# dmsuehir/unet_distributed

Hardware: AMD Instinct MI355X
Metric: images/sec (whole node) 2D UNet BraTS 128×128×4 at 1/2/4/8 MI355X; Dice parity (higher is better)
Workload: dtype bf16; 1 GPU; model=unet2d-transposed (base 32, depth 4, 7760385 params), global_batch=1024, per_gpu_batch=1024, img_size=128, in_channels=4, parallelism=dp1, backend=native

## Files before the change

unet_distributed_amd/csrc/kernels/conv_epilogue.h:

```cpp
#pragma once
#include "common.h"
#include "conv_params.h"

namespace unet {

struct PixCoord {
  int n, d, h, w;
};

__device__ __forceinline__ PixCoord decompose(int q, int OD, int OH, int OW) {
  PixCoord c;
  c.w = q % OW;
  int t = q / OW;
  c.h = t % OH;
  t /= OH;
  c.d = t % OD;
  c.n = t / OD;
  return c;
}

enum { EPI_GENERIC = 0, EPI_FWD = 1, EPI_DGRAD = 2, EPI_STATS = 3, EPI_DGRAD_NORM = 4 };

template <int BM, int BN, int NTHR = 256>
constexpr int epi_lds_bytes() {
// ... 35 lines not shown
  return EPI_GENERIC;
}

template <int WM>
struct LinearTiles {
  __device__ static int base(int wm, int i) { return wm * WM + i * 16; }
};
template <int W, int RW, int TC, int NCS>
struct StripTiles {
  __device__ static int base(int wave, int i) {
    return ((wave / NCS) * RW + i / TC) * W + (wave % NCS) * 16 * TC + (i % TC) * 16;
  }
};

constexpr int kWaitVm0 = 0x0f70, kWaitLgkm0 = 0xc07f;
__device__ __forceinline__ void lds_barrier() {
  asm volatile("" ::: "memory");
  __builtin_amdgcn_s_waitcnt(kWaitLgkm0);
  __builtin_amdgcn_s_barrier();
  asm volatile("" ::: "memory");
}

template <int TN>
struct EpiConst {
  float bias[TN][4];
  float hw[8];
  float hb;
};

struct HeadWsum {
// ... 4 lines not shown
  float t[8];
  bool on;
};

template <int BM, int BN, int NTHR>
__device__ __forceinline__ void epi_mask_bits_load(const ConvFwdParams& p, const int m0, const int n0, const int tid,
                                                   uint32_t (&mb)[BM * (BN / 8) / NTHR]) {
  constexpr int CPR = BN / 8, NIT = BM * CPR / NTHR, RPI = NTHR / CPR;
  static_assert(BM * CPR % NTHR == 0 && NTHR % CPR == 0, "whole chunk passes");
  const int co = n0 + (tid % CPR) * 8, ml0 = tid / CPR;
#pragma unroll
  for (int it = 0; it < NIT; ++it)
    mb[it] = ((const uint8_t*)p.mask1)[((size_t)(m0 + ml0 + it * RPI) * p.D1 + co) >> 3];
}

template <int BM, int BN, int WM, int WN, int TM, int TN, int NTHR, int EPI = EPI_GENERIC,
          class MapM = LinearTiles<WM>, int SEGW = 0, int TROW = 0>
__device__ __forceinline__ HeadWsum conv_epilogue(const ConvFwdParams p, f32x4 (&acc)[TM][TN], char* smem,
                                                  const int m0, const int n0, const int M, const int wm,
                                                  const int wn, const int lane, const int tid,
                                                  const int pitch = 0, const int col0 = 0, const int stat_row = 0,
                                                  const EpiConst<TN>* ec = nullptr, const HeadT ht = HeadT{},
                                                  const uint32_t* pmb = nullptr) {
  HeadWsum hws;
#pragma unroll
  for (int k = 0; k < 3; ++k)
#pragma unroll
    for (int e = 0; e < 8; ++e) hws.s[k][e] = 0.f;
  hws.u = hws.v = hws.w = 0.f;
  auto qof = [&](int ml) -> int {
    if constexpr (SEGW > 0) return (m0 + ml / SEGW) * pitch + col0 + (ml % SEGW);
    else return m0 + ml;
  };
  constexpr bool ESWZ = BN == 32;
  constexpr int EPI_STRIDE = ESWZ ? 64 : (BN + 4) * 2;
  auto eoff = [](const int ml, const int chunk) -> int {
    return ESWZ ? ml * 64 + 16 * (chunk ^ ((ml >> 2) & 3)) : ml * EPI_STRIDE + 16 * chunk;
  };
  auto ehalf = [](const int ml, const int nl) -> int {
    return ESWZ ? ml * 64 + 16 * ((nl >> 3) ^ ((ml >> 2) & 3)) + ((2 * (nl & 7)) ^ (8 * ((ml >> 1) & 1)))
                : ml * EPI_STRIDE + 2 * nl;
  };
  auto eread = [&](const int ml, const int chunk) -> u32x4 {
    if constexpr (ESWZ) {
// ... 192 lines not shown
      *(u32x4*)(dst + (size_t)q * p.Cout + n) = gv;
      unpack8(gv, g);
#pragma unroll
      for (int e = 0; e < 8; ++e) {
        s1[e] += g[e];
        s2[e] = fmaf(g[e], z[e], s2[e]);
      }
    }
    stats_out(s1, s2, cb);
    return hws;
  }
  if constexpr (EPI == EPI_DGRAD && NCHUNK % NTHR == 0 && NTHR % CPR == 0) {
    constexpr int NIT = NCHUNK / NTHR, RPI = NTHR / CPR;
    const int cb = tid % CPR, ml0 = tid / CPR;
    const int n = n0 + cb * 8;
    const bool side1 = n < p.D1;
    const int rs = side1 ? p.D1 : p.Cout - p.D1;
    const int co = side1 ? n : n - p.D1;
    h16* dst = (h16*)(side1 ? p.dst1 : p.dst2);
    const h16* mk = (const h16*)(side1 ? p.mask1 : p.mask2);
    const bool mbit = (p.mask_bits >> (side1 ? 0 : 1)) & 1;
    u32x4 mv[NIT];
    uint32_t mb[NIT];
    if (mk && pmb) {
#pragma unroll
      for (int it = 0; it < NIT; ++it) mb[it] = pmb[it];
    } else if (mk) {
#pragma unroll
      for (int it = 0; it < NIT; ++it) {
        const int q = qof(ml0 + it * RPI);
        if (q < M) {
          if (mbit)
            mb[it] = ((const uint8_t*)mk)[((size_t)q * rs + co) >> 3];
          else
            mv[it] = *(const u32x4*)(mk + (size_t)q * rs + co);
        }
      }
    }
    const bool route = !pmb && p.route_gy != nullptr, d3 = p.OD > 1;
    u32x4 rg[NIT];
    uint32_t rc[NIT], rk[NIT];
    if (route) {
      const int cpp = p.Cout >> 3;
#pragma unroll
      for (int it = 0; it < NIT; ++it) {
        const int q = qof(ml0 + it * RPI);
        if (q < M) {
          const size_t pq = route_pix(p, q, rk[it]);
          rc[it] = p.pool_code[pq * cpp + (n >> 3)];
          rg[it] = *(const u32x4*)((const h16*)p.route_gy + pq * p.Cout + n);
        }
      }
    }
#pragma unroll
    for (int it = 0; it < NIT; ++it) {
      const int ml = ml0 + it * RPI;
      const int q = qof(ml);
      if (q >= M) continue;
      u32x4 v = eread(ml, cb);
      if (mk) v = (mbit || pmb) ? keep_bits(v, mb[it]) : keep_pos(v, mv[it]);
      if (route) {
        float o[8], gg[8];
        unpack8(v, o);
        unpack8(rg[it], gg);
        const uint32_t cw = rc[it];
#pragma unroll
        for (int e = 0; e < 8; ++e)
          if (route_hit(cw, e, rk[it], d3)) o[e] += gg[e];
        v = pack8(o);
      }
      *(u32x4*)(dst + (size_t)q * rs + co) = v;
    }
    return hws;
  }
  const int Dt = kShuffle ? (p.Cout >> p.shuffle) : 0;
  constexpr bool kHeadable = EPI == EPI_FWD && BN == 32 && NTHR % CPR == 0;
  const bool kHead = kHeadable && p.head_w != nullptr;
  float hw[8], hb = 0.f;
  constexpr int HIT = kHeadable ? NCHUNK / NTHR : 1;
  static_assert(!kHeadable || (NCHUNK % NTHR == 0 && HIT % CPR == 0 && HIT <= 8), "fused head tiling");
  float hz[HIT];
  int hq[HIT];
#pragma unroll
  for (int k = 0; k < HIT; ++k) {
    hz[k] = 0.f;
    hq[k] = M;
  }
  if (kHeadable && kHead) {
#pragma unroll
    for (int e = 0; e < 8; ++e) hw[e] = ec ? ec->hw[e] : p.head_w[(tid % CPR) * 8 + e];
    hb = ec ? ec->hb : p.head_b[0];
  }
  constexpr int NITER = (NCHUNK + NTHR - 1) / NTHR;
  constexpr int UNR = kHeadable ? NITER : 2;
#pragma unroll UNR
  for (int it = 0; it < NITER; ++it) {
    const int c = tid + it * NTHR;
    if (NCHUNK % NTHR && c >= NCHUNK) break;
    const int ml = c / CPR, cb = c % CPR;
    const int q = qof(ml);
    if (q >= M) continue;
    const int n = n0 + cb * 8;
    u32x4 v = eread(ml, cb);
    size_t off;
    h16* dst;
    const void* mk;
    bool mbit = false;
    if (EPI == EPI_FWD || EPI == EPI_STATS) {
      off = (size_t)q * p.Cout + n;
      dst = (h16*)p.dst1;
      mk = nullptr;
    } else if (kShuffle) {
      const int tap = n / Dt, co = n - tap * Dt;
      const PixCoord pc = decompose(q, p.OD, p.OH, p.OW);
      int td = 0, th, tw;
      if (p.shuffle == 3) {
// ... 13 lines not shown
      mbit = p.mask_bits & 1;
    } else if (n < p.D1) {
      off = (size_t)q * p.D1 + n;
      dst = (h16*)p.dst1;
      mk = p.mask1;
      mbit = p.mask_bits & 1;
    } else {
      off = (size_t)q * (p.Cout - p.D1) + (n - p.D1);
      dst = (h16*)p.dst2;
      mk = p.mask2;
      mbit = (p.mask_bits >> 1) & 1;
    }
    if (EPI != EPI_FWD && EPI != EPI_STATS && mk) {
      v = mbit ? keep_bits(v, ((const uint8_t*)mk)[off >> 3]) : keep_pos(v, *(const u32x4*)((const h16*)mk + off));
    }
    if (!(kHeadable && kHead && p.head_nostore)) *(u32x4*)(dst + off) = v;
    if (EPI == EPI_FWD && p.relu_bits) p.relu_bits[off >> 3] = (uint8_t)pos_bits_relu(v);
    if (G && p.relu_bits) p.relu_bits[off >> 3] = (uint8_t)pos_bits(v);
    if constexpr (kHeadable) {
      if (kHead) {
        float f[8];
        unpack8(v, f);
        float z = 0.f;
#pragma unroll
        for (int e = 0; e < 8; ++e) z += f[e] * hw[e];
        z += __shfl_xor(z, 1, 64);
        z += __shfl_xor(z, 2, 64);
        hz[it] = z + hb;
        hq[it] = q;
        if (ht.on) {
          const float zl = z + hb;
          const float pr = __builtin_amdgcn_rcpf(1.f + __expf(-zl));
          const float tv = ht.t[it];
          const float vv = pr * (1.f - pr), uu = tv * vv, ww = pr - tv;
#pragma unroll
          for (int e = 0; e < 8; ++e) {
            hws.s[0][e] = fmaf(uu, f[e], hws.s[0][e]);
            hws.s[1][e] = fmaf(vv, f[e], hws.s[1][e]);
            hws.s[2][e] = fmaf(ww, f[e], hws.s[2][e]);
          }
          if (cb == 0) {
            hws.u += uu;
            hws.v += vv;
            hws.w += ww;
          }
// ... 1 lines not shown
      }
    }
  }
  if constexpr (kHeadable) {
    if (kHead) {
      const int cb = tid % CPR;
#pragma unroll
      for (int k = 0; k < HIT / CPR; ++k) {
        float z = hz[CPR * k];
        int q = hq[CPR * k];
#pragma unroll
        for (int r = 1; r < CPR; ++r) {
          z = cb == r ? hz[CPR * k + r] : z;
          q = cb == r ? hq[CPR * k + r] : q;
        }
        if (q < M) p.head_logit[q] = z;
      }
    }
  }
  if constexpr (EPI == EPI_FWD && TROW > 0 && (BM / TROW) % 2 == 0 && TROW % 2 == 0) {
    if (p.pool_dst) {
      constexpr int PC = TROW / 2, NP = (BM / TROW / 2) * PC * CPR;
      const int Wp = p.OW >> 1, cpp = p.Cout >> 3;
      h16* pdst = (h16*)p.pool_dst;
      for (int k = tid; k < NP; k += NTHR) {
        const int cb = k % CPR, pp = k / CPR;
        const int pr = pp / PC, pc = pp - pr * PC;
        const int ml00 = 2 * pr * TROW + 2 * pc;
        const int q00 = qof(ml00);
        if (q00 >= M) continue;
        int32_t key[8];
#pragma unroll
        for (int e = 0; e < 8; ++e) key[e] = INT32_MIN;
#pragma unroll
        for (int kk = 0; kk < 4; ++kk) {
          const int ml = ml00 + (kk >> 1) * TROW + (kk & 1);
          const u32x4 v = eread(ml, cb);
#pragma unroll
          for (int e = 0; e < 4; ++e) {
            key[2 * e] = max(key[2 * e], (int32_t)((v[e] << 16) | (3u - kk)));
            key[2 * e + 1] = max(key[2 * e + 1], (int32_t)((v[e] & 0xffff0000u) | (3u - kk)));
          }
        }
        uint32_t w = 0;
        u32x4 mv;
#pragma unroll
        for (int e = 0; e < 8; ++e)
          w |= ((3u - ((uint32_t)key[e] & 3u)) << (2 * e)) | ((key[e] > 3 ? 1u : 0u) << (24 + e));
#pragma unroll
        for (int e = 0; e < 4; ++e)
          mv[e] = ((uint32_t)key[2 * e] >> 16) | ((uint32_t)key[2 * e + 1] & 0xffff0000u);
        const int grow = q00 / p.OW, gcol = q00 - grow * p.OW;
        const size_t pq = (size_t)(grow >> 1) * Wp + (gcol >> 1);
        *(u32x4*)(pdst + pq * p.Cout + n0 + cb * 8) = mv;
        p.pool_code[pq * cpp + (n0 >> 3) + cb] = w;
      }
    }
  }
  return hws;
}

}
```

unet_distributed_amd/csrc/kernels/conv_win.h:

```cpp
#pragma once
#include "common.h"
#include "conv_params.h"
#include "conv_epilogue.h"
#include "head_grad.h"
#include <type_traits>

namespace unet {

enum { GEO_2D = 0, GEO_SEG = 1, GEO_3D = 2 };

inline int win_bn(const ConvFwdParams& p) {
  if (p.tile == 12) return 64;
  if (p.tile == 6) return 32;
  const int W = p.OW > 128 ? 128 : p.OW;
  return (p.Cout % 64 == 0 && W <= 64 && !p.head_w) ? 64 : 32;
}
inline int win_bm(const ConvFwdParams& p) {
  const int W = p.OW > 128 ? 128 : p.OW;
  return (W == 16 || win_bn(p) == 64) ? 256 : 512;
}
inline int win_rows(const ConvFwdParams& p) {
  const int W = p.OW > 128 ? 128 : p.OW;
  return win_bm(p) / W;
}
// ... 523 lines not shown
#pragma unroll
    for (int k = 0; k < 3; ++k)
#pragma unroll
      for (int e = 0; e < 8; ++e) red[wave * 100 + k * 32 + lane * 8 + e] = hws.s[k][e];
  }
  if (lane == 0) {
    red[wave * 100 + 96] = hws.u;
    red[wave * 100 + 97] = hws.v;
    red[wave * 100 + 98] = hws.w;
    red[wave * 100 + 99] = 0.f;
  }
  __syncthreads();
  if (tid < 100) row[tid] = (red[tid] + red[100 + tid]) + (red[200 + tid] + red[300 + tid]);
}

template <int EPI, int XF, int GEO = GEO_2D>
__global__ void __launch_bounds__(NTHR, 2) conv_win_pf_kernel(const ConvFwdParams p) {
  static_assert(XF == 0 || (XF == 3 && EPI == EPI_DGRAD && GEO == GEO_2D) || (XF == 1 && GEO == GEO_2D),
                "plain source, head-on-load data gradient or normalise on load");
  static_assert(GEO == GEO_2D || GEO == GEO_SEG, "2D rows");
  constexpr bool SEG = GEO == GEO_SEG;
  constexpr int W = 128, R = 4, BM = 512, BN = 32, ROWB = PF_ROWB;
  constexpr int TC = 2, NCS = 4, RW = 4, TM = RW * TC, TN = 2, WMP = BM / 4;
  using Map = StripTiles<W, RW, TC, NCS>;
  __shared__ __attribute__((aligned(1024))) char smem[PF_XB + PF_WB];
  char* Xs = smem;
  char* Ws = smem + PF_XB;
  const int tid = threadIdx.x, lane = tid & 63, wave = __builtin_amdgcn_readfirstlane(tid >> 6);
  const int H = p.OH;
  const int Wf = SEG ? p.OW : W;
  const int nseg = SEG ? p.OW / W : 1;
  const int rows_total = p.N * H;
  const int M = rows_total * Wf;
  const int nwin = rows_total / R * nseg;
// ... 3 lines not shown
  constexpr int OOB = 0x7fffffff;
  const char* src = (const char*)p.src1;

  u32x4 hv[PF_CPT], ev = {0u, 0u, 0u, 0u};
  const int gl_t = tid * 16;
  const int lds_t = (1 + (tid >> 2)) * 64 + 16 * ((tid & 3) ^ (((1 + (tid >> 2)) >> 1) & 3));
  constexpr int NSL = 6 * PF_HWP, HJ = (NSL + NTHR - 1) / NTHR;
  float hpr[HJ], htv[HJ];
  uint32_t hbits[HJ];
  HeadGradCtx hctx{};
  if constexpr (XF == 3) hctx = head_grad_ctx(p.hg);
  float xan[8], xbn[8];
  int pf_g0 = 0;
  bool pf_top = false, pf_bot = false;
  constexpr bool HWS = EPI == EPI_FWD && !SEG;
  float tnext[HWS ? 8 : 1];
  auto load_halo = [&](const int w) {
    const int tmw = p.rev ? nwin - 1 - w : w;
    const int g0 = (tmw / nseg) * R, col0 = (tmw % nseg) * W;
    if constexpr (HWS) {
      if (p.head_ws) {
#pragma unroll
        for (int it = 0; it < 8; ++it) tnext[it] = bits2f(((const uint16_t*)p.head_t)[g0 * W + (tid >> 2) + 64 * it]);
      }
    }
    if constexpr (XF == 3) {
      const bool top_in = (g0 % H) != 0, bot_in = ((g0 + R) % H) != 0;
#pragma unroll
      for (int j = 0; j < HJ; ++j) {
        const int sl = tid + NTHR * j;
        const int hr = sl / PF_HWP, hc = sl - hr * PF_HWP;
        const int gr = g0 - 1 + hr, col = hc - 1;
        const bool ok = sl < NSL && (hr > 0 || top_in) && (hr < R + 1 || bot_in) &&
                        (unsigned)gr < (unsigned)rows_total && (unsigned)col < (unsigned)W;
        const int pix = ok ? gr * W + col : 0;
        hpr[j] = p.hg.prob[pix];
        htv[j] = bits2f(((const uint16_t*)p.hg.t)[pix]);
        hbits[j] = ok ? ((const uint32_t*)p.hg.bits)[pix] : 0u;
// ... 4 lines not shown
    const bool top_in = (g0 % H) != 0, bot_in = ((g0 + R) % H) != 0;
    if constexpr (XF == 1) {
      const size_t cs = (size_t)(g0 / H) * p.xcs + (tid & 3) * 8;
#pragma unroll
      for (int e = 0; e < 8; ++e) {
        xan[e] = p.xa[cs + e];
        xbn[e] = p.xb[cs + e];
      }
      pf_g0 = g0;
      pf_top = top_in;
      pf_bot = bot_in;
    }
    const __amdgpu_buffer_rsrc_t rs =
        __builtin_amdgcn_make_buffer_rsrc((void*)(src + (size_t)grow0 * Wf * 64), (short)0, OOB, 0x00020000);
    const int rowoff = ((g0 - 1 - grow0) * Wf + col0) * 64;
#pragma unroll
    for (int c = 0; c < PF_CPT; ++c) {
      const int hr = c >> 1;
      const bool ok = (hr > 0 || top_in) && (hr < R + 1 || bot_in) && (unsigned)(g0 - 1 + hr) < (unsigned)rows_total;
      hv[c] = __builtin_amdgcn_raw_buffer_load_b128(rs, ok ? rowoff + hr * Wf * 64 + (c & 1) * 4096 + gl_t : OOB, 0, 0);
    }
    if constexpr (SEG) {
      const int hr = tid >> 3, col = ((tid >> 2) & 1) ? col0 + W : col0 - 1;
      const bool ok = tid < 48 && (hr > 0 || top_in) && (hr < R + 1 || bot_in) &&
                      (unsigned)(g0 - 1 + hr) < (unsigned)rows_total && (unsigned)col < (unsigned)Wf;
      ev = __builtin_amdgcn_raw_buffer_load_b128(
          rs, ok ? ((g0 - 1 + hr - grow0) * Wf + col) * 64 + (tid & 3) * 16 : OOB, 0, 0);
    }
  };
  auto store_halo = [&]() {
    if constexpr (XF == 3) {
#pragma unroll
      for (int j = 0; j < HJ; ++j) {
        const int sl = tid + NTHR * j;
        if (sl >= NSL) continue;
// ... 24 lines not shown
          unpack8(v, f);
#pragma unroll
          for (int e = 0; e < 8; ++e) f[e] = fmaxf(fmaf(xan[e], f[e], xbn[e]), 0.f);
          v = pack8(f);
          if (p.xout && hr >= 1 && hr <= R)
            *(u32x4*)((h16*)p.xout + ((size_t)gr * W + (tid >> 2) + 64 * (c & 1)) * 32 + (tid & 3) * 8) = v;
        }
        *(u32x4*)(Xs + lds_t + hr * ROWB + (c & 1) * 4096) = v;
      }
    } else {
#pragma unroll
      for (int c = 0; c < PF_CPT; ++c) *(u32x4*)(Xs + lds_t + (c >> 1) * ROWB + (c & 1) * 4096) = hv[c];
    }
    if (tid < 48) *(u32x4*)(Xs + (tid >> 3) * ROWB + ((tid >> 2) & 1) * 129 * 64 + 16 * (tid & 3)) = ev;
  };
  load_halo(w_lo);
  {
    const __amdgpu_buffer_rsrc_t rsw = __builtin_amdgcn_make_buffer_rsrc((void*)p.wgt, (short)0, OOB, 0x00020000);
    const int lslot = lane >> 2;
    const int lchunk = (lane & 3) ^ ((lslot >> 1) & 3);
    const int wl = (lslot * p.Kpad + lchunk * 8) * 2;
    constexpr int WI = 9 * BN / 16;
#pragma unroll
    for (int q = 0; q < (WI + 3) / 4; ++q) {
      const int k = wave + 4 * q;
      if (k < WI) {
        const int tap = k / (BN / 16), nb = (k % (BN / 16)) * 16;
        __builtin_amdgcn_raw_ptr_buffer_load_lds(rsw, (__attribute__((address_space(3))) void*)(Ws + k * 1024), 16,
                                                 (nb * p.Kpad + tap * 32) * 2 + wl, 0, 0, 0);
      }
// ... 4 lines not shown
#pragma unroll
  for (int j = 0; j < TN; ++j)
#pragma unroll
    for (int r = 0; r < 4; ++r)
      ec.bias[j][r] = (EPI != EPI_DGRAD && EPI != EPI_DGRAD_NORM && p.bias) ? p.bias[16 * j + 4 * fsub + r] : 0.f;
#pragma unroll
  for (int e = 0; e < 8; ++e) ec.hw[e] = (EPI == EPI_FWD && p.head_w) ? p.head_w[(tid % 4) * 8 + e] : 0.f;
  ec.hb = (EPI == EPI_FWD && p.head_w) ? p.head_b[0] : 0.f;
  HeadWsum hws;
#pragma unroll
  for (int k = 0; k < 3; ++k)
#pragma unroll
    for (int e = 0; e < 8; ++e) hws.s[k][e] = 0.f;
  hws.u = hws.v = hws.w = 0.f;
  HeadT ht;
  ht.on = HWS && p.head_ws;
#pragma unroll
  for (int it = 0; it < 8; ++it) ht.t[it] = HWS ? tnext[it] : 0.f;
  store_halo();
  __syncthreads();

  const int r0 = (wave / NCS) * RW, c0 = (wave % NCS) * 16 * TC;
  int xbase[3];
#pragma unroll
  for (int dw = 0; dw < 3; ++dw) {
    const int hc = fr + dw;
    xbase[dw] = r0 * ROWB + c0 * 64 + hc * 64 + 16 * (fsub ^ ((hc >> 1) & 3));
  }
  const int wbase = fr * 64 + 16 * (fsub ^ ((fr >> 1) & 3));
  for (int w = w_lo; w < w_hi; ++w) {
    const int tm = p.rev ? nwin - 1 - w : w;
    const int g0 = (tm / nseg) * R, col0 = (tm % nseg) * W;
    if (w + 1 < w_hi) load_halo(w + 1);
    f32x4 acc[TM][TN];
#pragma unroll
    for (int i = 0; i < TM; ++i)
#pragma unroll
      for (int j = 0; j < TN; ++j) acc[i][j] = (f32x4){0.f, 0.f, 0.f, 0.f};
#pragma unroll
    for (int dw = 0; dw < 3; ++dw) {
      h16x8 wf[3][TN];
#pragma unroll
      for (int dh = 0; dh < 3; ++dh)
#pragma unroll
        for (int j = 0; j < TN; ++j) wf[dh][j] = *(const h16x8*)(Ws + ((3 * dh + dw) * BN + 16 * j) * 64 + wbase);
#pragma unroll
      for (int hr = 0; hr < RW + 2; ++hr) {
#pragma unroll
// ... 2 lines not shown
#pragma unroll
          for (int dh = 0; dh < 3; ++dh) {
            const int ri = hr - dh;
            if (ri < 0 || ri >= RW) continue;
#pragma unroll
            for (int j = 0; j < TN; ++j) acc[ri * TC + ci][j] = mfma16(wf[dh][j], xf, acc[ri * TC + ci][j]);
          }
        }
      }
    }
    __syncthreads();
    if constexpr (SEG)
      conv_epilogue<BM, BN, WMP, BN, TM, TN, NTHR, EPI, Map, W, W>(p, acc, smem, g0, 0, M, wave, 0, lane, tid, Wf,
                                                                    col0, tm, &ec);
    else {
      const HeadWsum r = conv_epilogue<BM, BN, WMP, BN, TM, TN, NTHR, EPI, Map, 0, W>(
          p, acc, smem, g0 * W, 0, M, wave, 0, lane, tid, 0, 0, tm, &ec, ht);
      if constexpr (HWS) {
#pragma unroll
        for (int k = 0; k < 3; ++k)
#pragma unroll
          for (int e = 0; e < 8; ++e) hws.s[k][e] += r.s[k][e];
        hws.u += r.u;
        hws.v += r.v;
        hws.w += r.w;
      }
    }
    if (w + 1 < w_hi) {
      __syncthreads();
      store_halo();
      if constexpr (HWS) {
#pragma unroll
        for (int it = 0; it < 8; ++it) ht.t[it] = tnext[it];
      }
      __syncthreads();
    }
  }
  if constexpr (EPI == EPI_FWD && !SEG) {
    if (p.head_ws) head_ws_store(hws, smem, wave, lane, tid, p.head_ws + (size_t)blockIdx.x * 100);
  }
}

template <int W, bool CONCAT, int EPI, bool DZ = false>
__global__ void __launch_bounds__(NTHR, 2) conv_win_cp_kernel(const ConvFwdParams p) {
  constexpr int BN = 64, BM = 256, R = BM / W, HR = R + 2;
  constexpr int HWP = W + 4, ROWB = HWP * 64;
  constexpr int NSLOT = HR * HWP;
  constexpr int XB = (NSLOT + 15) / 16 * 1024, WB = 9 * BN * 64;
  constexpr int XG = (NSLOT * 4 + NTHR - 1) / NTHR;
  constexpr int WG = 9 * BN * 4 / NTHR;
  constexpr int EPIB = (EPI == EPI_STATS || EPI == EPI_DGRAD_NORM) ? epi_lds_bytes<BM, BN>() : BM * (BN + 4) * 2;
  constexpr int KB = DZ ? 3 * CP_DZ_MAXC * 4 : 0;
  constexpr int LDS_BYTES = (XB + WB + KB > EPIB) ? XB + WB + KB : EPIB;
  constexpr int WMP = BM / 4, TM = WMP / 16, TN = BN / 16;
// ... 347 lines not shown
    default: UNET_LAUNCH((conv_win_cp128_kernel<GEO, CC, EPI_GENERIC>), dim3(grid), dim3(NTHR), 0, s, p); break;     \
  }
  if (cc) {
    CP1_EPI(true)
  } else {
    CP1_EPI(false)
  }
#undef CP1_EPI
  return launch_status();
}

hipError_t launch_win_cp128(const ConvFwdParams& p, hipStream_t s) {
  return (p.KD == 3) ? launch_win_cp128_g<GEO_3D>(p, s) : launch_win_cp128_g<GEO_2D>(p, s);
}

template <int KS, int EPI>
__global__ void __launch_bounds__(NTHR, 2) conv_win_pfu_kernel(const ConvFwdParams p) {
  static_assert(EPI == EPI_FWD || EPI == EPI_STATS, "persistent tconv-on-load epilogues");
  constexpr int W = 128, R = 2, HR = R + 2, BM = 256, BN = 32, ROWB = PF_ROWB;
  constexpr int TC = 2, NCS = 4, RW = 2, TM = RW * TC, TN = 2, WMP = BM / 4;
  constexpr int CW = W / 2, PB = CW / 16, Cc = KS * 32;
  constexpr int XB = HR * ROWB, WB = 9 * BN * 64;
  static_assert(BM * 64 + 4 * 2 * BN * 4 <= XB, "epilogue staging aliases the halo image");
  using Map = StripTiles<W, RW, TC, NCS>;
  __shared__ __attribute__((aligned(1024))) char smem[XB + 2 * WB];
  char* Xs = smem;
  char* Wu = smem + XB;
  char* Wk = smem + XB + WB;
  const int tid = threadIdx.x, lane = tid & 63, wave = __builtin_amdgcn_readfirstlane(tid >> 6);
  const int fsub = lane >> 4, fr = lane & 15;
  const int H = p.OH;
  const int rows_total = p.N * H;
  const int M = rows_total * W;
// ... 34 lines not shown
  }
  float bs[8];
#pragma unroll
  for (int i = 0; i < 8; ++i) bs[i] = p.ut.b[8 * fsub + i];
  EpiConst<TN> ec;
#pragma unroll
  for (int j = 0; j < TN; ++j)
#pragma unroll
    for (int r = 0; r < 4; ++r) ec.bias[j][r] = p.bias ? p.bias[16 * j + 4 * fsub + r] : 0.f;
#pragma unroll
  for (int e = 0; e < 8; ++e) ec.hw[e] = 0.f;
  ec.hb = 0.f;

  h16x8 xb[PB][KS];
  bool xin = false;
  auto load_coarse = [&](const int w) {
    const int g0 = (p.rev ? nwin - 1 - w : w) * R;
    const bool top_in = (g0 % H) != 0, bot_in = ((g0 + R) % H) != 0;
    const int hr = wave;
    xin = (hr > 0 || top_in) && (hr < R + 1 || bot_in) && (unsigned)(g0 - 1 + hr) < (unsigned)rows_total;
    const int crow = (g0 >> 1) - 1 + cq;
    const h16* rp = (const h16*)p.ut.x + ((size_t)(xin ? crow : 0) * CW + fr) * Cc + 8 * fsub;
#pragma unroll
    for (int pb = 0; pb < PB; ++pb)
#pragma unroll
      for (int ks = 0; ks < KS; ++ks) xb[pb][ks] = *(const h16x8*)(rp + (size_t)(16 * pb) * Cc + 32 * ks);
  };
  u32x4 sv[8];
  uint32_t sok = 0;
  float s2a[8], s2b[8];
  const int lds_t = (1 + (tid >> 2)) * 64 + 16 * ((tid & 3) ^ (((1 + (tid >> 2)) >> 1) & 3));
  auto load_skip = [&](const int w) {
    const int g0 = (p.rev ? nwin - 1 - w : w) * R;
    const int grow0 = (g0 / H) * H;
    const bool top_in = (g0 % H) != 0, bot_in = ((g0 + R) % H) != 0;
    const __amdgpu_buffer_rsrc_t rs =
        __builtin_amdgcn_make_buffer_rsrc((void*)((const char*)p.src2 + (size_t)grow0 * W * 64), (short)0, OOB, 0x00020000);
    const int rowoff = (g0 - 1 - grow0) * W * 64;
    sok = 0;
#pragma unroll
    for (int c = 0; c < 8; ++c) {
      const int hr = c >> 1;
      const bool ok = (hr > 0 || top_in) && (hr < R + 1 || bot_in) && (unsigned)(g0 - 1 + hr) < (unsigned)rows_total;
      sok |= (ok ? 1u : 0u) << c;
      sv[c] = __builtin_amdgcn_raw_buffer_load_b128(rs, ok ? rowoff + hr * W * 64 + (c & 1) * 4096 + tid * 16 : OOB, 0, 0);
    }
    if (p.x2a) {
      const size_t cs = (size_t)(g0 / H) * p.x2cs + (tid & 3) * 8;
#pragma unroll
      for (int e = 0; e < 8; ++e) {
        s2a[e] = p.x2a[cs + e];
        s2b[e] = p.x2b[cs + e];
      }
    }
  };
  const int tsel = (fr >> 2) & 1;
  auto form_u = [&]() {
    char* xrow = Xs + wave * ROWB;
#pragma unroll
    for (int pb = 0; pb < PB; ++pb) {
      u32x4 pk[2] = {(u32x4){0u, 0u, 0u, 0u}, (u32x4){0u, 0u, 0u, 0u}};
      if (xin) {
// ... 6 lines not shown
            for (int ks = 0; ks < KS; ++ks) a = mfma16(wa[tw][j][ks], xb[pb][ks], a);
            pk[tw][2 * j] = pack2h(a[0] + bs[4 * j], a[1] + bs[4 * j + 1]);
            pk[tw][2 * j + 1] = pack2h(a[2] + bs[4 * j + 2], a[3] + bs[4 * j + 3]);
          }
      }
#pragma unroll
      for (int s = 0; s < 2; ++s) {
        const int tw = s ^ tsel;
        const int hc = 2 * (16 * pb + fr) + tw + 1;
        *(u32x4*)(xrow + hc * 64 + 16 * (fsub ^ ((hc >> 1) & 3))) = tw ? pk[1] : pk[0];
      }
    }
    if (lane < 8) *(u32x4*)(xrow + ((lane >> 2) ? W + 1 : 0) * 64 + 16 * (lane & 3)) = (u32x4){0u, 0u, 0u, 0u};
  };
  auto store_skip = [&]() {
    if (p.x2a) {
#pragma unroll
      for (int c = 0; c < 8; ++c) {
        if (!((sok >> c) & 1u)) continue;
        float f[8];
        unpack8(sv[c], f);
#pragma unroll
        for (int e = 0; e < 8; ++e) f[e] = fmaxf(fmaf(s2a[e], f[e], s2b[e]), 0.f);
        sv[c] = pack8(f);
      }
    }
#pragma unroll
    for (int c = 0; c < 8; ++c) *(u32x4*)(Xs + lds_t + (c >> 1) * ROWB + (c & 1) * 4096) = sv[c];
    if (tid < 32) *(u32x4*)(Xs + (tid >> 3) * ROWB + ((tid >> 2) & 1) * 129 * 64 + 16 * (tid & 3)) = (u32x4){0u, 0u, 0u, 0u};
  };

// ... 20 lines not shown
        for (int ci = 0; ci < TC; ++ci) {
          const h16x8 xf = *(const h16x8*)(Xs + xbase[dw] + hr * ROWB + ci * 16 * 64);
#pragma unroll
          for (int dh = 0; dh < 3; ++dh) {
            const int ri = hr - dh;
            if (ri < 0 || ri >= RW) continue;
#pragma unroll
            for (int j = 0; j < TN; ++j) acc[ri * TC + ci][j] = mfma16(wf[dh][j], xf, acc[ri * TC + ci][j]);
          }
        }
      }
    }
  };
  load_coarse(w_lo);
  load_skip(w_lo);
  for (int w = w_lo; w < w_hi; ++w) {
    const int tm = p.rev ? nwin - 1 - w : w;
    const int g0 = tm * R;
#pragma unroll
    for (int i = 0; i < TM; ++i)
#pragma unroll
      for (int j = 0; j < TN; ++j) acc[i][j] = (f32x4){0.f, 0.f, 0.f, 0.f};
    form_u();
    if (w + 1 < w_hi) load_coarse(w + 1);
    __syncthreads();
    chunk_mfmas(Wu);
    __syncthreads();
    store_skip();
    if (w + 1 < w_hi) load_skip(w + 1);
    __syncthreads();
    chunk_mfmas(Wk);
    __syncthreads();
    conv_epilogue<BM, BN, WMP, BN, TM, TN, NTHR, EPI, Map, 0, W>(p, acc, smem, g0 * W, 0, M, wave, 0, lane, tid, 0, 0,
                                                                  tm, &ec);
    __syncthreads();
  }
}

hipError_t launch_win_pfu(const ConvFwdParams& p, hipStream_t s) {
  const int grid = win_grid(p);
  const bool st = conv_epi_mode(p) == EPI_STATS;
  if (p.ut.C == 64 && st)
    UNET_LAUNCH((conv_win_pfu_kernel<2, EPI_STATS>), dim3(grid), dim3(NTHR), 0, s, p);
  else if (p.ut.C == 64)
    UNET_LAUNCH((conv_win_pfu_kernel<2, EPI_FWD>), dim3(grid), dim3(NTHR), 0, s, p);
  else if (st)
    UNET_LAUNCH((conv_win_pfu_kernel<1, EPI_STATS>), dim3(grid), dim3(NTHR), 0, s, p);
  else
    UNET_LAUNCH((conv_win_pfu_kernel<1, EPI_FWD>), dim3(grid), dim3(NTHR), 0, s, p);
  return launch_status();
}

hipError_t launch_win_pf(const ConvFwdParams& p, hipStream_t s) {
  const int grid = win_grid(p);
  if (p.OW > 128) {
    switch (conv_epi_mode(p)) {
      case EPI_FWD: UNET_LAUNCH((conv_win_pf_kernel<EPI_FWD, 0, GEO_SEG>), dim3(grid), dim3(NTHR), 0, s, p); break;
      case EPI_DGRAD: UNET_LAUNCH((conv_win_pf_kernel<EPI_DGRAD, 0, GEO_SEG>), dim3(grid), dim3(NTHR), 0, s, p); break;
// ... 1 lines not shown
      case EPI_DGRAD_NORM:
        UNET_LAUNCH((conv_win_pf_kernel<EPI_DGRAD_NORM, 0, GEO_SEG>), dim3(grid), dim3(NTHR), 0, s, p);
        break;
      default: UNET_LAUNCH((conv_win_pf_kernel<EPI_GENERIC, 0, GEO_SEG>), dim3(grid), dim3(NTHR), 0, s, p); break;
    }
    return launch_status();
  }
  if (p.xform) {
    if (conv_epi_mode(p) == EPI_STATS)
      UNET_LAUNCH((conv_win_pf_kernel<EPI_STATS, 1>), dim3(grid), dim3(NTHR), 0, s, p);
    else if (conv_epi_mode(p) == EPI_GENERIC)
      UNET_LAUNCH((conv_win_pf_kernel<EPI_GENERIC, 1>), dim3(grid), dim3(NTHR), 0, s, p);
    else
      return hipErrorInvalidValue;
    return launch_status();
  }
  switch (conv_epi_mode(p)) {
    case EPI_FWD: UNET_LAUNCH((conv_win_pf_kernel<EPI_FWD, 0>), dim3(grid), dim3(NTHR), 0, s, p); break;
    case EPI_DGRAD:
      if (p.hg.prob)
        UNET_LAUNCH((conv_win_pf_kernel<EPI_DGRAD, 3>), dim3(grid), dim3(NTHR), 0, s, p);
      else
        UNET_LAUNCH((conv_win_pf_kernel<EPI_DGRAD, 0>), dim3(grid), dim3(NTHR), 0, s, p);
      break;
    case EPI_STATS: UNET_LAUNCH((conv_win_pf_kernel<EPI_STATS, 0>), dim3(grid), dim3(NTHR), 0, s, p); break;
    case EPI_DGRAD_NORM: UNET_LAUNCH((conv_win_pf_kernel<EPI_DGRAD_NORM, 0>), dim3(grid), dim3(NTHR), 0, s, p); break;
    default: UNET_LAUNCH((conv_win_pf_kernel<EPI_GENERIC, 0>), dim3(grid), dim3(NTHR), 0, s, p); break;
  }
  return launch_status();
}
// ... 188 lines not shown
```

Before: 49940 images/sec.

## Specialise windowed conv epilogues into fixed compile-time forms for common layer configs

Adds a FORM template parameter that fixes at compile time which epilogue features (ReLU bitmask, 2x2 pool, fused head, gradient routing) are active and asserts full tiles, removing runtime pointer checks and bounds tests. The host picks these specialised kernels when the parameters match. The prefetch loop now always issues loads, dummy and clamped via a max-offset trick, so control flow has no branches, and head targets are loaded later as packed 32-bit words. It adds more kernel instantiations and assumes whole windows, which risks correctness if the dispatch conditions miss a case, and the extra dummy loads cost some bandwidth.

```diff
diff --git a/unet_distributed_amd/csrc/kernels/conv_epilogue.h b/unet_distributed_amd/csrc/kernels/conv_epilogue.h
--- a/unet_distributed_amd/csrc/kernels/conv_epilogue.h
+++ b/unet_distributed_amd/csrc/kernels/conv_epilogue.h
@@ -73,6 +73,8 @@
 };
 
 constexpr int kWaitVm0 = 0x0f70, kWaitLgkm0 = 0xc07f;
+constexpr int vm_wait(const int n) { return (n & 15) | ((n >> 4) << 14) | 0x0f70; }
+static_assert(vm_wait(0) == kWaitVm0 && vm_wait(63) == 0xcf7f, "gfx9 s_waitcnt encoding");
 __device__ __forceinline__ void lds_barrier() {
   asm volatile("" ::: "memory");
   __builtin_amdgcn_s_waitcnt(kWaitLgkm0);
@@ -107,8 +109,18 @@
     mb[it] = ((const uint8_t*)p.mask1)[((size_t)(m0 + ml0 + it * RPI) * p.D1 + co) >> 3];
 }
 
+enum { EF_FULL = 1, EF_FIXED = 2, EF_BITS = 4, EF_POOL = 8, EF_HEAD = 16, EF_ROUTE = 32 };
+template <int BM, int BN, int NTHR, int EPI, int TROW, int FORM>
+constexpr int epi_store_count() {
+  if (!(FORM & EF_FIXED)) return 0;
+  constexpr int CPR = BN / 8, NIT = BM * CPR / NTHR;
+  if (EPI == EPI_DGRAD) return NIT;
+  return ((FORM & EF_HEAD) ? NIT / CPR : NIT) + ((FORM & EF_BITS) ? NIT : 0) +
+         ((FORM & EF_POOL) ? 2 * ((BM / TROW / 2) * (TROW / 2) * CPR / NTHR) : 0);
+}
+
 template <int BM, int BN, int WM, int WN, int TM, int TN, int NTHR, int EPI = EPI_GENERIC,
-          class MapM = LinearTiles<WM>, int SEGW = 0, int TROW = 0>
+          class MapM = LinearTiles<WM>, int SEGW = 0, int TROW = 0, int FORM = 0>
 __device__ __forceinline__ HeadWsum conv_epilogue(const ConvFwdParams p, f32x4 (&acc)[TM][TN], char* smem,
                                                   const int m0, const int n0, const int M, const int wm,
                                                   const int wn, const int lane, const int tid,
@@ -121,6 +133,9 @@
 #pragma unroll
     for (int e = 0; e < 8; ++e) hws.s[k][e] = 0.f;
   hws.u = hws.v = hws.w = 0.f;
+  constexpr bool FULL = (FORM & EF_FULL) != 0, FIXED = (FORM & EF_FIXED) != 0;
+  static_assert(!FIXED || (FULL && SEGW == 0 && (EPI == EPI_FWD || EPI == EPI_DGRAD)), "fixed forms: whole 2D windows");
+  static_assert(!FIXED || EPI != EPI_DGRAD || (FORM & EF_BITS), "fixed data-gradient forms take a 1-bit mask");
   auto qof = [&](int ml) -> int {
     if constexpr (SEGW > 0) return (m0 + ml / SEGW) * pitch + col0 + (ml % SEGW);
     else return m0 + ml;
@@ -343,22 +358,22 @@
     constexpr int NIT = NCHUNK / NTHR, RPI = NTHR / CPR;
     const int cb = tid % CPR, ml0 = tid / CPR;
     const int n = n0 + cb * 8;
-    const bool side1 = n < p.D1;
+    const bool side1 = FIXED || n < p.D1;
     const int rs = side1 ? p.D1 : p.Cout - p.D1;
     const int co = side1 ? n : n - p.D1;
     h16* dst = (h16*)(side1 ? p.dst1 : p.dst2);
     const h16* mk = (const h16*)(side1 ? p.mask1 : p.mask2);
-    const bool mbit = (p.mask_bits >> (side1 ? 0 : 1)) & 1;
+    const bool mbit = FIXED || ((p.mask_bits >> (side1 ? 0 : 1)) & 1);
     u32x4 mv[NIT];
     uint32_t mb[NIT];
-    if (mk && pmb) {
+    if ((FIXED || mk) && pmb) {
 #pragma unroll
       for (int it = 0; it < NIT; ++it) mb[it] = pmb[it];
-    } else if (mk) {
+    } else if (FIXED || mk) {
 #pragma unroll
       for (int it = 0; it < NIT; ++it) {
         const int q = qof(ml0 + it * RPI);
-        if (q < M) {
+        if (FULL || q < M) {
           if (mbit)
             mb[it] = ((const uint8_t*)mk)[((size_t)q * rs + co) >> 3];
           else
@@ -366,7 +381,8 @@
         }
       }
     }
-    const bool route = !pmb && p.route_gy != nullptr, d3 = p.OD > 1;
+    const bool route = FIXED ? (FORM & EF_ROUTE) != 0 : (!pmb && p.route_gy != nullptr);
+    const bool d3 = !FIXED && p.OD > 1;
     u32x4 rg[NIT];
     uint32_t rc[NIT], rk[NIT];
     if (route) {
@@ -374,7 +390,7 @@
 #pragma unroll
       for (int it = 0; it < NIT; ++it) {
         const int q = qof(ml0 + it * RPI);
-        if (q < M) {
+        if (FULL || q < M) {
           const size_t pq = route_pix(p, q, rk[it]);
           rc[it] = p.pool_code[pq * cpp + (n >> 3)];
           rg[it] = *(const u32x4*)((const h16*)p.route_gy + pq * p.Cout + n);
@@ -385,9 +401,9 @@
     for (int it = 0; it < NIT; ++it) {
       const int ml = ml0 + it * RPI;
       const int q = qof(ml);
-      if (q >= M) continue;
+      if (!FULL && q >= M) continue;
       u32x4 v = eread(ml, cb);
-      if (mk) v = (mbit || pmb) ? keep_bits(v, mb[it]) : keep_pos(v, mv[it]);
+      if (FIXED || mk) v = (mbit || pmb) ? keep_bits(v, mb[it]) : keep_pos(v, mv[it]);
       if (route) {
         float o[8], gg[8];
         unpack8(v, o);
@@ -404,7 +420,11 @@
   }
   const int Dt = kShuffle ? (p.Cout >> p.shuffle) : 0;
   constexpr bool kHeadable = EPI == EPI_FWD && BN == 32 && NTHR % CPR == 0;
-  const bool kHead = kHeadable && p.head_w != nullptr;
+  static_assert(!FIXED || EPI != EPI_FWD || kHeadable || !(FORM & EF_HEAD), "fixed head form: a headable tile");
+  const bool kHead = FIXED ? (FORM & EF_HEAD) != 0 : (kHeadable && p.head_w != nullptr);
+  const bool kNoStore = FIXED ? (FORM & EF_HEAD) != 0 : (kHeadable && kHead && p.head_nostore);
+  const bool kBitsF = FIXED ? (FORM & EF_BITS) != 0 : (p.relu_bits != nullptr);
+  const bool kHws = FIXED ? (FORM & EF_HEAD) != 0 : ht.on;
   float hw[8], hb = 0.f;
   constexpr int HIT = kHeadable ? NCHUNK / NTHR : 1;
   static_assert(!kHeadable || (NCHUNK % NTHR == 0 && HIT % CPR == 0 && HIT <= 8), "fused head tiling");
@@ -428,7 +448,7 @@
     if (NCHUNK % NTHR && c >= NCHUNK) break;
     const int ml = c / CPR, cb = c % CPR;
     const int q = qof(ml);
-    if (q >= M) continue;
+    if (!FULL && q >= M) continue;
     const int n = n0 + cb * 8;
     u32x4 v = eread(ml, cb);
     size_t off;
@@ -472,21 +492,27 @@
     if (EPI != EPI_FWD && EPI != EPI_STATS && mk) {
       v = mbit ? keep_bits(v, ((const uint8_t*)mk)[off >> 3]) : keep_pos(v, *(const u32x4*)((const h16*)mk + off));
     }
-    if (!(kHeadable && kHead && p.head_nostore)) *(u32x4*)(dst + off) = v;
-    if (EPI == EPI_FWD && p.relu_bits) p.relu_bits[off >> 3] = (uint8_t)pos_bits_relu(v);
+    if (!kNoStore) *(u32x4*)(dst + off) = v;
+    if (EPI == EPI_FWD && kBitsF) p.relu_bits[off >> 3] = (uint8_t)pos_bits_relu(v);
     if (G && p.relu_bits) p.relu_bits[off >> 3] = (uint8_t)pos_bits(v);
     if constexpr (kHeadable) {
       if (kHead) {
         float f[8];
         unpack8(v, f);
         float z = 0.f;
-#pragma unroll
-        for (int e = 0; e < 8; ++e) z += f[e] * hw[e];
+        if constexpr (FIXED) {
+#pragma clang fp contract(off)
+#pragma unroll
+          for (int e = 0; e < 8; ++e) z += f[e] * hw[e];
+        } else {
+#pragma unroll
+          for (int e = 0; e < 8; ++e) z += f[e] * hw[e];
+        }
         z += __shfl_xor(z, 1, 64);
         z += __shfl_xor(z, 2, 64);
         hz[it] = z + hb;
-        hq[it] = q;
-        if (ht.on) {
+        if constexpr (!FULL) hq[it] = q;
+        if (kHws) {
           const float zl = z + hb;
           const float pr = __builtin_amdgcn_rcpf(1.f + __expf(-zl));
           const float tv = ht.t[it];
@@ -518,21 +544,22 @@
           z = cb == r ? hz[CPR * k + r] : z;
           q = cb == r ? hq[CPR * k + r] : q;
         }
-        if (q < M) p.head_logit[q] = z;
+        if constexpr (FULL) q = qof((tid + (CPR * k + cb) * NTHR) / CPR);
+        if (FULL || q < M) p.head_logit[q] = z;
       }
     }
   }
   if constexpr (EPI == EPI_FWD && TROW > 0 && (BM / TROW) % 2 == 0 && TROW % 2 == 0) {
-    if (p.pool_dst) {
+    if (FIXED ? (FORM & EF_POOL) != 0 : p.pool_dst != nullptr) {
       constexpr int PC = TROW / 2, NP = (BM / TROW / 2) * PC * CPR;
       const int Wp = p.OW >> 1, cpp = p.Cout >> 3;
       h16* pdst = (h16*)p.pool_dst;
-      for (int k = tid; k < NP; k += NTHR) {
+      auto pool_px = [&](const int k) {
         const int cb = k % CPR, pp = k / CPR;
         const int pr = pp / PC, pc = pp - pr * PC;
         const int ml00 = 2 * pr * TROW + 2 * pc;
         const int q00 = qof(ml00);
-        if (q00 >= M) continue;
+        if (!FULL && q00 >= M) return;
         int32_t key[8];
 #pragma unroll
         for (int e = 0; e < 8; ++e) key[e] = INT32_MIN;
@@ -558,6 +585,12 @@
         const size_t pq = (size_t)(grow >> 1) * Wp + (gcol >> 1);
         *(u32x4*)(pdst + pq * p.Cout + n0 + cb * 8) = mv;
         p.pool_code[pq * cpp + (n0 >> 3) + cb] = w;
+      };
+      if constexpr (FULL && NP % NTHR == 0) {
+#pragma unroll
+        for (int kp = 0; kp < NP / NTHR; ++kp) pool_px(tid + kp * NTHR);
+      } else {
+        for (int k = tid; k < NP; k += NTHR) pool_px(k);
       }
     }
   }
diff --git a/unet_distributed_amd/csrc/kernels/conv_win.h b/unet_distributed_amd/csrc/kernels/conv_win.h
--- a/unet_distributed_amd/csrc/kernels/conv_win.h
+++ b/unet_distributed_amd/csrc/kernels/conv_win.h
@@ -561,10 +561,13 @@
   if (tid < 100) row[tid] = (red[tid] + red[100 + tid]) + (red[200 + tid] + red[300 + tid]);
 }
 
-template <int EPI, int XF, int GEO = GEO_2D>
+template <int EPI, int XF, int GEO = GEO_2D, int FORM = 0>
 __global__ void __launch_bounds__(NTHR, 2) conv_win_pf_kernel(const ConvFwdParams p) {
   static_assert(XF == 0 || (XF == 3 && EPI == EPI_DGRAD && GEO == GEO_2D) || (XF == 1 && GEO == GEO_2D),
                 "plain source, head-on-load data gradient or normalise on load");
+  static_assert(FORM == 0 || (XF == 0 && GEO == GEO_2D), "fixed epilogue forms: the plain 128-wide window");
+  constexpr bool FIXED = (FORM & EF_FIXED) != 0;
+  const bool head_ws_on = FIXED ? (FORM & EF_HEAD) != 0 : (p.head_ws != nullptr);
   static_assert(GEO == GEO_2D || GEO == GEO_SEG, "2D rows");
   constexpr bool SEG = GEO == GEO_SEG;
   constexpr int W = 128, R = 4, BM = 512, BN = 32, ROWB = PF_ROWB;
@@ -598,14 +601,20 @@
   int pf_g0 = 0;
   bool pf_top = false, pf_bot = false;
   constexpr bool HWS = EPI == EPI_FWD && !SEG;
-  float tnext[HWS ? 8 : 1];
-  auto load_halo = [&](const int w) {
+  uint32_t tnext[HWS ? 8 : 1];
+  constexpr bool TLATE = HWS && FIXED && (FORM & EF_HEAD) != 0;
+  auto load_targets = [&](const int w) {
+    const int g0 = (p.rev ? nwin - 1 - w : w) * R;
+#pragma unroll
+    for (int it = 0; it < 8; ++it) tnext[it] = ((const uint32_t*)p.head_t)[(g0 * W + (tid >> 2) + 64 * it) >> 1];
+  };
+  auto load_halo = [&](const int w, const bool live = true) {
     const int tmw = p.rev ? nwin - 1 - w : w;
     const int g0 = (tmw / nseg) * R, col0 = (tmw % nseg) * W;
-    if constexpr (HWS) {
-      if (p.head_ws) {
-#pragma unroll
-        for (int it = 0; it < 8; ++it) tnext[it] = bits2f(((const uint16_t*)p.head_t)[g0 * W + (tid >> 2) + 64 * it]);
+    if constexpr (HWS && !TLATE) {
+      if (head_ws_on) {
+#pragma unroll
+        for (int it = 0; it < 8; ++it) tnext[it] = ((const uint16_t*)p.head_t)[g0 * W + (tid >> 2) + 64 * it];
       }
     }
     if constexpr (XF == 3) {
@@ -640,11 +649,20 @@
     const __amdgpu_buffer_rsrc_t rs =
         __builtin_amdgcn_make_buffer_rsrc((void*)(src + (size_t)grow0 * Wf * 64), (short)0, OOB, 0x00020000);
     const int rowoff = ((g0 - 1 - grow0) * Wf + col0) * 64;
+    const unsigned rows_live = live ? (unsigned)rows_total : 0u;
 #pragma unroll
     for (int c = 0; c < PF_CPT; ++c) {
       const int hr = c >> 1;
-      const bool ok = (hr > 0 || top_in) && (hr < R + 1 || bot_in) && (unsigned)(g0 - 1 + hr) < (unsigned)rows_total;
-      hv[c] = __builtin_amdgcn_raw_buffer_load_b128(rs, ok ? rowoff + hr * Wf * 64 + (c & 1) * 4096 + gl_t : OOB, 0, 0);
+      const bool ok = (hr > 0 || top_in) && (hr < R + 1 || bot_in) && (unsigned)(g0 - 1 + hr) < rows_live;
+      int off = rowoff + hr * Wf * 64 + (c & 1) * 4096 + gl_t;
+      if constexpr (FIXED) {
+        int lim = ok ? INT32_MIN : OOB;
+        asm volatile("" : "+s"(lim));
+        off = max(off, lim);
+      } else {
+        off = ok ? off : OOB;
+      }
+      hv[c] = __builtin_amdgcn_raw_buffer_load_b128(rs, off, 0, 0);
     }
     if constexpr (SEG) {
       const int hr = tid >> 3, col = ((tid >> 2) & 1) ? col0 + W : col0 - 1;
@@ -699,6 +717,7 @@
     }
     if (tid < 48) *(u32x4*)(Xs + (tid >> 3) * ROWB + ((tid >> 2) & 1) * 129 * 64 + 16 * (tid & 3)) = ev;
   };
+  if constexpr (TLATE) load_targets(w_lo);
   load_halo(w_lo);
   {
     const __amdgpu_buffer_rsrc_t rsw = __builtin_amdgcn_make_buffer_rsrc((void*)p.wgt, (short)0, OOB, 0x00020000);
@@ -733,9 +752,9 @@
     for (int e = 0; e < 8; ++e) hws.s[k][e] = 0.f;
   hws.u = hws.v = hws.w = 0.f;
   HeadT ht;
-  ht.on = HWS && p.head_ws;
-#pragma unroll
-  for (int it = 0; it < 8; ++it) ht.t[it] = HWS ? tnext[it] : 0.f;
+  ht.on = HWS && head_ws_on;
+#pragma unroll
+  for (int it = 0; it < 8; ++it) ht.t[it] = (HWS && !TLATE) ? bits2f((uint16_t)tnext[it]) : 0.f;
   store_halo();
   __syncthreads();
 
@@ -750,7 +769,11 @@
   for (int w = w_lo; w < w_hi; ++w) {
     const int tm = p.rev ? nwin - 1 - w : w;
     const int g0 = (tm / nseg) * R, col0 = (tm % nseg) * W;
-    if (w + 1 < w_hi) load_halo(w + 1);
+    const bool more = w + 1 < w_hi;
+    if constexpr (FIXED)
+      load_halo(more ? w + 1 : w, more);
+    else if (more)
+      load_halo(w + 1);
     f32x4 acc[TM][TN];
 #pragma unroll
     for (int i = 0; i < TM; ++i)
@@ -783,7 +806,15 @@
       conv_epilogue<BM, BN, WMP, BN, TM, TN, NTHR, EPI, Map, W, W>(p, acc, smem, g0, 0, M, wave, 0, lane, tid, Wf,
                                                                     col0, tm, &ec);
     else {
-      const HeadWsum r = conv_epilogue<BM, BN, WMP, BN, TM, TN, NTHR, EPI, Map, 0, W>(
+      if constexpr (TLATE) {
+#pragma unroll
+        for (int it = 0; it < 8; ++it) {
+          uint32_t r = tnext[it];
+          asm volatile("" : "+v"(r));
+          ht.t[it] = bits2f((uint16_t)(r >> (16 * ((tid >> 2) & 1))));
+        }
+      }
+      const HeadWsum r = conv_epilogue<BM, BN, WMP, BN, TM, TN, NTHR, EPI, Map, 0, W, FORM>(
           p, acc, smem, g0 * W, 0, M, wave, 0, lane, tid, 0, 0, tm, &ec, ht);
       if constexpr (HWS) {
 #pragma unroll
@@ -795,18 +826,19 @@
         hws.w += r.w;
       }
     }
-    if (w + 1 < w_hi) {
+    if (FIXED || more) {
       __syncthreads();
       store_halo();
-      if constexpr (HWS) {
-#pragma unroll
-        for (int it = 0; it < 8; ++it) ht.t[it] = tnext[it];
+      if constexpr (TLATE) load_targets(more ? w + 1 : w);
+      if constexpr (HWS && !TLATE) {
+#pragma unroll
+        for (int it = 0; it < 8; ++it) ht.t[it] = bits2f((uint16_t)tnext[it]);
       }
       __syncthreads();
     }
   }
   if constexpr (EPI == EPI_FWD && !SEG) {
-    if (p.head_ws) head_ws_store(hws, smem, wave, lane, tid, p.head_ws + (size_t)blockIdx.x * 100);
+    if (head_ws_on) head_ws_store(hws, smem, wave, lane, tid, p.head_ws + (size_t)blockIdx.x * 100);
   }
 }
 
@@ -1184,9 +1216,11 @@
   return (p.KD == 3) ? launch_win_cp128_g<GEO_3D>(p, s) : launch_win_cp128_g<GEO_2D>(p, s);
 }
 
-template <int KS, int EPI>
+template <int KS, int EPI, int FORM = 0>
 __global__ void __launch_bounds__(NTHR, 2) conv_win_pfu_kernel(const ConvFwdParams p) {
   static_assert(EPI == EPI_FWD || EPI == EPI_STATS, "persistent tconv-on-load epilogues");
+  static_assert(FORM == 0 || EPI == EPI_FWD, "fixed epilogue forms (conv_win_pf_kernel's): bias + ReLU");
+  constexpr bool FIXED = (FORM & EF_FIXED) != 0;
   constexpr int W = 128, R = 2, HR = R + 2, BM = 256, BN = 32, ROWB = PF_ROWB;
   constexpr int TC = 2, NCS = 4, RW = 2, TM = RW * TC, TN = 2, WMP = BM / 4;
   constexpr int CW = W / 2, PB = CW / 16, Cc = KS * 32;
@@ -1251,11 +1285,11 @@
 
   h16x8 xb[PB][KS];
   bool xin = false;
-  auto load_coarse = [&](const int w) {
+  auto load_coarse = [&](const int w, const bool live = true) {
     const int g0 = (p.rev ? nwin - 1 - w : w) * R;
     const bool top_in = (g0 % H) != 0, bot_in = ((g0 + R) % H) != 0;
     const int hr = wave;
-    xin = (hr > 0 || top_in) && (hr < R + 1 || bot_in) && (unsigned)(g0 - 1 + hr) < (unsigned)rows_total;
+    xin = live && (hr > 0 || top_in) && (hr < R + 1 || bot_in) && (unsigned)(g0 - 1 + hr) < (unsigned)rows_total;
     const int crow = (g0 >> 1) - 1 + cq;
     const h16* rp = (const h16*)p.ut.x + ((size_t)(xin ? crow : 0) * CW + fr) * Cc + 8 * fsub;
 #pragma unroll
@@ -1267,7 +1301,7 @@
   uint32_t sok = 0;
   float s2a[8], s2b[8];
   const int lds_t = (1 + (tid >> 2)) * 64 + 16 * ((tid & 3) ^ (((1 + (tid >> 2)) >> 1) & 3));
-  auto load_skip = [&](const int w) {
+  auto load_skip = [&](const int w, const bool live = true) {
     const int g0 = (p.rev ? nwin - 1 - w : w) * R;
     const int grow0 = (g0 / H) * H;
     const bool top_in = (g0 % H) != 0, bot_in = ((g0 + R) % H) != 0;
@@ -1278,11 +1312,20 @@
 #pragma unroll
     for (int c = 0; c < 8; ++c) {
       const int hr = c >> 1;
-      const bool ok = (hr > 0 || top_in) && (hr < R + 1 || bot_in) && (unsigned)(g0 - 1 + hr) < (unsigned)rows_total;
+      const bool ok = live && (hr > 0 || top_in) && (hr < R + 1 || bot_in) &&
+                      (unsigned)(g0 - 1 + hr) < (unsigned)rows_total;
       sok |= (ok ? 1u : 0u) << c;
-      sv[c] = __builtin_amdgcn_raw_buffer_load_b128(rs, ok ? rowoff + hr * W * 64 + (c & 1) * 4096 + tid * 16 : OOB, 0, 0);
-    }
-    if (p.x2a) {
+      int off = rowoff + hr * W * 64 + (c & 1) * 4096 + tid * 16;
+      if constexpr (FIXED) {
+        int lim = ok ? INT32_MIN : OOB;
+        asm volatile("" : "+s"(lim));
+        off = max(off, lim);
+      } else {
+        off = ok ? off : OOB;
+      }
+      sv[c] = __builtin_amdgcn_raw_buffer_load_b128(rs, off, 0, 0);
+    }
+    if (!FIXED && p.x2a) {
       const size_t cs = (size_t)(g0 / H) * p.x2cs + (tid & 3) * 8;
 #pragma unroll
       for (int e = 0; e < 8; ++e) {
@@ -1319,7 +1362,7 @@
     if (lane < 8) *(u32x4*)(xrow + ((lane >> 2) ? W + 1 : 0) * 64 + 16 * (lane & 3)) = (u32x4){0u, 0u, 0u, 0u};
   };
   auto store_skip = [&]() {
-    if (p.x2a) {
+    if (!FIXED && p.x2a) {
 #pragma unroll
       for (int c = 0; c < 8; ++c) {
         if (!((sok >> c) & 1u)) continue;
@@ -1370,6 +1413,7 @@
   };
   load_coarse(w_lo);
   load_skip(w_lo);
+  if constexpr (FIXED) __builtin_amdgcn_s_waitcnt(kWaitVm0);
   for (int w = w_lo; w < w_hi; ++w) {
     const int tm = p.rev ? nwin - 1 - w : w;
     const int g0 = tm * R;
@@ -1377,20 +1421,36 @@
     for (int i = 0; i < TM; ++i)
 #pragma unroll
       for (int j = 0; j < TN; ++j) acc[i][j] = (f32x4){0.f, 0.f, 0.f, 0.f};
+    const bool more = w + 1 < w_hi;
     form_u();
-    if (w + 1 < w_hi) load_coarse(w + 1);
+    if (FIXED || more) load_coarse(more ? w + 1 : w, more);
     __syncthreads();
     chunk_mfmas(Wu);
     __syncthreads();
     store_skip();
-    if (w + 1 < w_hi) load_skip(w + 1);
+    if (FIXED || more) load_skip(more ? w + 1 : w, more);
     __syncthreads();
     chunk_mfmas(Wk);
     __syncthreads();
-    conv_epilogue<BM, BN, WMP, BN, TM, TN, NTHR, EPI, Map, 0, W>(p, acc, smem, g0 * W, 0, M, wave, 0, lane, tid, 0, 0,
-                                                                  tm, &ec);
+    conv_epilogue<BM, BN, WMP, BN, TM, TN, NTHR, EPI, Map, 0, W, FORM>(p, acc, smem, g0 * W, 0, M, wave, 0, lane, tid,
+                                                                        0, 0, tm, &ec);
     __syncthreads();
   }
+}
+
+constexpr int kFormBits = EF_FULL | EF_FIXED | EF_BITS;
+constexpr int kFormPool = kFormBits | EF_POOL, kFormHead = kFormBits | EF_HEAD, kFormRoute = kFormBits | EF_ROUTE;
+inline int win_epi_form(const ConvFwdParams& p) {
+  const int ep = conv_epi_mode(p);
+  if (ep == EPI_FWD && p.dst1 && p.relu_bits && !p.head_w && !p.head_ws && !p.head_nostore)
+    return p.pool_dst ? (p.pool_code ? kFormPool : 0) : kFormBits;
+  if (ep == EPI_FWD && p.relu_bits && p.head_w && p.head_b && p.head_logit && p.head_ws && p.head_t &&
+      ((uintptr_t)p.head_t & 3) == 0 && p.head_nostore && !p.pool_dst)
+    return kFormHead;
+  if (ep == EPI_DGRAD && p.dst1 && p.D1 == p.Cout && p.mask1 && (p.mask_bits & 1) && p.route_gy && p.pool_code &&
+      p.OD == 1)
+    return kFormRoute;
+  return 0;
 }
 
 hipError_t launch_win_pfu(const ConvFwdParams& p, hipStream_t s) {
@@ -1398,6 +1458,8 @@
   const bool st = conv_epi_mode(p) == EPI_STATS;
   if (p.ut.C == 64 && st)
     UNET_LAUNCH((conv_win_pfu_kernel<2, EPI_STATS>), dim3(grid), dim3(NTHR), 0, s, p);
+  else if (p.ut.C == 64 && win_epi_form(p) == kFormBits && !p.x2a)
+    UNET_LAUNCH((conv_win_pfu_kernel<2, EPI_FWD, kFormBits>), dim3(grid), dim3(NTHR), 0, s, p);
   else if (p.ut.C == 64)
     UNET_LAUNCH((conv_win_pfu_kernel<2, EPI_FWD>), dim3(grid), dim3(NTHR), 0, s, p);
   else if (st)
@@ -1429,6 +1491,19 @@
     else
       return hipErrorInvalidValue;
     return launch_status();
+  }
+  switch (win_epi_form(p)) {
+    case kFormPool:
+      UNET_LAUNCH((conv_win_pf_kernel<EPI_FWD, 0, GEO_2D, kFormPool>), dim3(grid), dim3(NTHR), 0, s, p);
+      return launch_status();
+    case kFormHead:
+      UNET_LAUNCH((conv_win_pf_kernel<EPI_FWD, 0, GEO_2D, kFormHead>), dim3(grid), dim3(NTHR), 0, s, p);
+      return launch_status();
+    case kFormRoute:
+      if (p.hg.prob) break;
+      UNET_LAUNCH((conv_win_pf_kernel<EPI_DGRAD, 0, GEO_2D, kFormRoute>), dim3(grid), dim3(NTHR), 0, s, p);
+      return launch_status();
+    default: break;
   }
   switch (conv_epi_mode(p)) {
     case EPI_FWD: UNET_LAUNCH((conv_win_pf_kernel<EPI_FWD, 0>), dim3(grid), dim3(NTHR), 0, s, p); break;
```

Result: no change. 49760 images/sec, median of 2 (-0.4%).
